# jongwon-jay-lee/llmss

Hardware: AMD Instinct MI355X
Metric: output_tokens_per_sec (higher is better)
Workload: dtype bf16

## Files before the change

### llmss_amd/csrc/common.h

```cpp
#pragma once
#include <hip/hip_runtime.h>
#include <hip/hip_bf16.h>
#include <stdint.h>
#include <algorithm>
#include <stdexcept>
#include <string>

#define LLMSS_WAVE 64

typedef unsigned short bf16_t;
typedef unsigned short __attribute__((ext_vector_type(8))) u16x8;
typedef unsigned short __attribute__((ext_vector_type(4))) u16x4;
typedef short __attribute__((ext_vector_type(8))) s16x8;
typedef short __attribute__((ext_vector_type(4))) s16x4;
typedef float __attribute__((ext_vector_type(4))) f32x4;
typedef float __attribute__((ext_vector_type(16))) f32x16;
typedef float __attribute__((ext_vector_type(2))) f32x2;
typedef unsigned int __attribute__((ext_vector_type(4))) u32x4;
typedef unsigned int __attribute__((ext_vector_type(2))) u32x2;

#define LDS_AS __attribute__((address_space(3)))

__device__ __forceinline__ float bf2f(bf16_t x) { return __uint_as_float(((unsigned)x) << 16); }

// ... 70 lines not shown
__device__ __forceinline__ float apply_act(float x, int act) {
  switch (act) {
    case ACT_GELU_TANH: return gelu_tanh(x);
    case ACT_GELU: return gelu_erf(x);
    case ACT_RELU: return fmaxf(x, 0.f);
    default: return x;
  }
}

__device__ __forceinline__ int xcd_remap(int orig, int nwg) {
  const int q = nwg >> 3, r = nwg & 7, xcd = orig & 7, idx = orig >> 3;
  return (xcd < r ? xcd * (q + 1) : r * (q + 1) + (xcd - r) * q) + idx;
}

__device__ __forceinline__ __amdgpu_buffer_rsrc_t uniform_rsrc(const void* p, int64_t bytes) {
  const uint64_t a = reinterpret_cast<uint64_t>(p);
  const uint32_t lo = __builtin_amdgcn_readfirstlane((uint32_t)a);
  const uint32_t hi = __builtin_amdgcn_readfirstlane((uint32_t)(a >> 32));
  const int n = __builtin_amdgcn_readfirstlane((int)(bytes < 0x7fffffff ? bytes : 0x7fffffff));
  return __builtin_amdgcn_make_buffer_rsrc(reinterpret_cast<void*>(((uint64_t)hi << 32) | lo), (short)0, n,
                                           0x00020000);
}

template <bool P32>
__device__ __forceinline__ f32x2 swap_pair(float x) {
  unsigned a = __builtin_bit_cast(unsigned, x), b = a;
  if constexpr (P32) asm volatile("s_nop 1\n\tv_permlane32_swap_b32 %0, %1" : "+v"(a), "+v"(b));
  else asm volatile("s_nop 1\n\tv_permlane16_swap_b32 %0, %1" : "+v"(a), "+v"(b));
  return f32x2{__builtin_bit_cast(float, a), __builtin_bit_cast(float, b)};
}
__device__ __forceinline__ float xor16_max(float x) { const f32x2 r = swap_pair<false>(x); return fmaxf(r[0], r[1]); }
__device__ __forceinline__ float xor32_max(float x) { const f32x2 r = swap_pair<true>(x); return fmaxf(r[0], r[1]); }
__device__ __forceinline__ float xor16_sum(float x) { const f32x2 r = swap_pair<false>(x); return r[0] + r[1]; }
__device__ __forceinline__ float xor32_sum(float x) { const f32x2 r = swap_pair<true>(x); return r[0] + r[1]; }

struct TileWork {
  int m0, n0, z;
};
__device__ __forceinline__ TileWork tile_work(int ntm, int ntn, int bm, int bn) {
  const int G = gridDim.x * gridDim.y;
  const int w = xcd_remap(blockIdx.y * gridDim.x + blockIdx.x, G);
  const int per = ntm * ntn;
  const int z = w / per, t = w - z * per;
  const int nt = t / ntm;
  return {(t - nt * ntm) * bm, nt * bn, z};
}

struct QkvEpi {
  const int64_t* pos;
  const float* cos_t;
  const float* sin_t;
  bf16_t* kc;
  bf16_t* vc;
  const int64_t* slot;
  int nh, nkv, D, rot, block_size, style, do_rope;
  unsigned char* mxq;
  unsigned char* mxs;
};

__device__ __forceinline__ int mx_block_exp(float amax) {
  const uint32_t b = __float_as_uint(amax / 448.f);
  int e = (int)((b >> 23) & 255) - 127 + ((b & 0x7fffffu) != 0u);
  return e < -126 ? -126 : (e > 126 ? 126 : e);
}

template <int BN>
struct EpiImg {
  static constexpr bool SWZ = BN % 32 == 0;
  static constexpr int LDW = SWZ ? BN : BN + 4;
  __device__ static __forceinline__ int at(int r, int c) { return r * LDW + (SWZ ? (c ^ (((r >> 2) & 1) << 4)) : c); }
  __device__ static __forceinline__ f32x4 ld4(const float* ct, int r, int c) {
    return *reinterpret_cast<const f32x4*>(ct + at(r, c));
  }
  __device__ static __forceinline__ void ld8(const float* ct, int r, int c, float (&x)[8]) {
    const int key = (threadIdx.x >> 3) & 1;
    const f32x4 a = ld4(ct, r, c + 4 * key), b = ld4(ct, r, c + 4 * (key ^ 1));
#pragma unroll
    for (int i = 0; i < 4; ++i) {
      x[i] = key ? b[i] : a[i];
      x[4 + i] = key ? a[i] : b[i];
    }
  }
};

template <int BN, int NTHR, int R>
__device__ __forceinline__ void qkv_store_chunk(const QkvEpi& e, const float* ct, int rows, int r0, int m0,
                                                int n0, int M, int N, bf16_t* __restrict__ Y, int64_t ldy,
                                                const bf16_t* __restrict__ bias) {
  constexpr int VPR = BN / 8, ITEMS = (R * VPR + NTHR - 1) / NTHR, G = ITEMS < 4 ? ITEMS : 4;
  const int D = e.D, nq = e.nh * D, nk = e.nkv * D, rh = e.rot >> 1;
  const bool rope = e.do_rope != 0;
#pragma unroll
  for (int i0 = 0; i0 < ITEMS; i0 += G) {
    int rr[G], cc[G], mm[G];
    bool ok[G];
    int64_t p[G], sl[G];
#pragma unroll
    for (int j = 0; j < G; ++j) {
      const int v = threadIdx.x + (i0 + j) * NTHR;
      rr[j] = v / VPR;
      cc[j] = (v - rr[j] * VPR) * 8;
      mm[j] = m0 + r0 + rr[j];
      ok[j] = i0 + j < ITEMS && rr[j] < rows && mm[j] < M && n0 + cc[j] < N;
      const int mc = min(mm[j], M - 1);
      p[j] = rope ? e.pos[mc] : 0;
      sl[j] = e.kc ? e.slot[mc] : -1;
    }
    f32x4 cs[G][2], sn[G][2];
#pragma unroll
    for (int j = 0; j < G; ++j) {
      if (rope) {
        const int n = n0 + cc[j], d = n % D;
        const bool lo = d < rh;
        int a = e.style == 1 ? (d >> 1) : (lo ? d : d - rh);
        a = (n < nq + nk && d < e.rot) ? a : 0;
        const float* cp = e.cos_t + p[j] * rh + a;
        const float* sp = e.sin_t + p[j] * rh + a;
        cs[j][0] = *reinterpret_cast<const f32x4*>(cp);
        sn[j][0] = *reinterpret_cast<const f32x4*>(sp);
        if (e.style != 1 && rh >= 8) {
          cs[j][1] = *reinterpret_cast<const f32x4*>(cp + 4);
          sn[j][1] = *reinterpret_cast<const f32x4*>(sp + 4);
        }
      }
    }
#pragma unroll
    for (int j = 0; j < G; ++j) {
      if (!ok[j]) continue;
      const int c = cc[j], n = n0 + c, d = n % D, m = mm[j];
      float x[8], y[8];
      EpiImg<BN>::ld8(ct, rr[j], c, x);
#pragma unroll
      for (int i = 0; i < 8; ++i) {
        x[i] = bf2f(f2bf(x[i] + (bias ? bf2f(bias[n + i]) : 0.f)));
        y[i] = x[i];
      }
      const bool is_v = n >= nq + nk;
      if (rope && !is_v && d < e.rot) {
        if (e.style == 1) {
#pragma unroll
          for (int i = 0; i < 4; ++i) {
            y[2 * i] = x[2 * i] * cs[j][0][i] - x[2 * i + 1] * sn[j][0][i];
            y[2 * i + 1] = x[2 * i + 1] * cs[j][0][i] + x[2 * i] * sn[j][0][i];
          }
        } else {
          const bool lo = d < rh;
          const int sh = lo ? rh : -rh;
          float xs[8];
          EpiImg<BN>::ld8(ct, rr[j], c + sh, xs);
#pragma unroll
          for (int i = 0; i < 8; ++i) {
            const float xp = bf2f(f2bf(xs[i] + (bias ? bf2f(bias[n + sh + i]) : 0.f)));
            const float cv = cs[j][i >> 2][i & 3], sv = sn[j][i >> 2][i & 3];
            y[i] = lo ? x[i] * cv - xp * sv : x[i] * cv + xp * sv;
          }
        }
      }
      u16x8 o;
#pragma unroll
      for (int i = 0; i < 8; ++i) o[i] = f2bf(y[i]);
      *reinterpret_cast<u16x8*>(Y + (int64_t)m * ldy + n) = o;
      if (n >= nq && sl[j] >= 0) {
        const int h = (n - (is_v ? nq + nk : nq)) / D;
        const int64_t row = ((sl[j] / e.block_size) * e.nkv + h) * (int64_t)e.block_size + sl[j] % e.block_size;
        *reinterpret_cast<u16x8*>((is_v ? e.vc : e.kc) + row * D + d) = o;
      }
    }
  }
}

template <int BN, int NTHR, int R>
__device__ __forceinline__ void img_store_rows(const float* ct, int rows, int r0, int m0, int n0, int M, int N,
                                               float* __restrict__ part, bf16_t* __restrict__ Y, int64_t ldy,
                                               const bf16_t* __restrict__ bias, int act, int glu, const QkvEpi& qe) {
  using Img = EpiImg<BN>;
  if (qe.D) {
    qkv_store_chunk<BN, NTHR, R>(qe, ct, rows, r0, m0, n0, M, N, Y, ldy, bias);
  } else if (part) {
    constexpr int VPR = BN / 4;
    for (int v = threadIdx.x; v < rows * VPR; v += NTHR) {
      const int r = v / VPR, c = (v - r * VPR) * 4;
      const int m = m0 + r0 + r, n = n0 + c;
      if (m >= M || n >= N) continue;
      const f32x4 val = Img::ld4(ct, r, c);
      float* dst = part + (int64_t)m * N + n;
      if (n + 3 < N && (N & 3) == 0) *reinterpret_cast<f32x4*>(dst) = val;
      else
        for (int j = 0; j < 4 && n + j < N; ++j) dst[j] = val[j];
    }
  } else if (glu && qe.mxq) {
    constexpr int VPR = BN / 16;
    static_assert(BN % 16 == 0, "SwiGLU tile");
    if constexpr (VPR % 4 == 0) {
      for (int v = threadIdx.x; v < rows * VPR; v += NTHR) {
        const int r = v / VPR, oc = (v - r * VPR) * 8;
        const int p = oc >> 4, j = oc & 15;
        const int cg = 32 * p + j, m = m0 + r0 + r, ng = n0 + cg;
        const bool ok = m < M && ng < N;
        float gx[8], ux[8], h[8];
        Img::ld8(ct, r, cg, gx);
        Img::ld8(ct, r, cg + 16, ux);
        float amax = 0.f;
#pragma unroll
        for (int e = 0; e < 8; ++e) {
          float gv = gx[e], uv = ux[e];
          if (bias && ok) { gv += bf2f(bias[ng + e]); uv += bf2f(bias[ng + 16 + e]); }
          h[e] = bf2f(f2bf(silu(gv) * uv));
          amax = fmaxf(amax, fabsf(h[e]));
        }
        amax = fmaxf(amax, __shfl_xor(amax, 1, 64));
        amax = fmaxf(amax, __shfl_xor(amax, 2, 64));
        const int ex = amax > 0.f ? mx_block_exp(amax) : 0;
        const float inv = __uint_as_float((uint32_t)(127 - ex) << 23);
        unsigned lo = 0, hi = 0;
        lo = __builtin_amdgcn_cvt_pk_fp8_f32(h[0] * inv, h[1] * inv, lo, false);
        lo = __builtin_amdgcn_cvt_pk_fp8_f32(h[2] * inv, h[3] * inv, lo, true);
        hi = __builtin_amdgcn_cvt_pk_fp8_f32(h[4] * inv, h[5] * inv, hi, false);
        hi = __builtin_amdgcn_cvt_pk_fp8_f32(h[6] * inv, h[7] * inv, hi, true);
        const int64_t oc_g = n0 / 2 + oc;
        if (ok) {
          *reinterpret_cast<uint2*>(qe.mxq + (int64_t)m * ldy + oc_g) = make_uint2(lo, hi);
          if ((v & 3) == 0) qe.mxs[(int64_t)m * (ldy / 32) + oc_g / 32] = (unsigned char)(ex + 127);
        }
      }
    }
  } else if (glu) {
    constexpr int VPR = BN / 16;
    for (int v = threadIdx.x; v < rows * VPR; v += NTHR) {
      const int r = v / VPR, oc = (v - r * VPR) * 8;
      const int p = oc >> 4, j = oc & 15;
      const int cg = 32 * p + j, m = m0 + r0 + r, ng = n0 + cg;
      if (m >= M || ng >= N) continue;
      u16x8 o;
      float gx[8], ux[8];
      Img::ld8(ct, r, cg, gx);
      Img::ld8(ct, r, cg + 16, ux);
#pragma unroll
      for (int e = 0; e < 8; ++e) {
        float gv = gx[e], uv = ux[e];
        if (bias) { gv += bf2f(bias[ng + e]); uv += bf2f(bias[ng + 16 + e]); }
        o[e] = f2bf(silu(gv) * uv);
      }
      bf16_t* dst = Y + (int64_t)m * ldy + n0 / 2 + oc;
      if (ng + 16 + 7 < N && (ldy & 7) == 0) *reinterpret_cast<u16x8*>(dst) = o;
      else
        for (int e = 0; e < 8 && ng + 16 + e < N; ++e) dst[e] = o[e];
    }
  } else {
    constexpr int VPR = BN / 8;
    for (int v = threadIdx.x; v < rows * VPR; v += NTHR) {
      const int r = v / VPR, c = (v - r * VPR) * 8;
      const int m = m0 + r0 + r, n = n0 + c;
      if (m >= M || n >= N) continue;
      u16x8 o;
      float xv[8];
      Img::ld8(ct, r, c, xv);
#pragma unroll
      for (int e = 0; e < 8; ++e) {
        float x = xv[e];
        if (bias && n + e < N) x += bf2f(bias[n + e]);
        o[e] = f2bf(apply_act(x, act));
      }
      bf16_t* dst = Y + (int64_t)m * ldy + n;
      if (n + 7 < N && (ldy & 7) == 0) *reinterpret_cast<u16x8*>(dst) = o;
      else
        for (int e = 0; e < 8 && n + e < N; ++e) dst[e] = o[e];
    }
  }
}

template <int BM, int BN, int MT, int NT, int NTHR, int LDSB>
__device__ __forceinline__ void tile_store_lds(const f32x4 (&acc)[MT][NT], char* lds, int wrow0, int wcol0, int m0,
                                               int n0, int M, int N, float* __restrict__ part,
                                               bf16_t* __restrict__ Y, int64_t ldy, const bf16_t* __restrict__ bias,
                                               int act, int glu, const QkvEpi& qe = QkvEpi{}) {
  using Img = EpiImg<BN>;
  constexpr int RMAX = LDSB / (Img::LDW * 4);
  constexpr int R = (RMAX >= BM ? BM : RMAX) / 16 * 16;
  static_assert(R >= 16, "LDS too small for a 16-row epilogue chunk");
  float* ct = reinterpret_cast<float*>(lds);
  const int lane = threadIdx.x & 63, li = lane & 15, g = lane >> 4;
  asm volatile("s_waitcnt lgkmcnt(0)" ::: "memory");
  __builtin_amdgcn_s_barrier();
  asm volatile("" ::: "memory");
  for (int r0 = 0; r0 < BM; r0 += R) {
#pragma unroll
    for (int mt = 0; mt < MT; ++mt) {
      const int rb = wrow0 + mt * 16;
      if (rb < r0 || rb >= r0 + R) continue;
#pragma unroll
      for (int i = 0; i < 4; ++i)
#pragma unroll
        for (int nt = 0; nt < NT; ++nt) ct[Img::at(rb - r0 + 4 * g + i, wcol0 + nt * 16 + li)] = acc[mt][nt][i];
    }
    asm volatile("s_waitcnt lgkmcnt(0)" ::: "memory");
    __builtin_amdgcn_s_barrier();
    asm volatile("" ::: "memory");
    const int rows = BM - r0 < R ? BM - r0 : R;
    img_store_rows<BN, NTHR, R>(ct, rows, r0, m0, n0, M, N, part, Y, ldy, bias, act, glu, qe);
    if (r0 + R < BM) {
      asm volatile("s_waitcnt lgkmcnt(0)" ::: "memory");
      __builtin_amdgcn_s_barrier();
      asm volatile("" ::: "memory");
    }
  }
}

template <int MT, int NT>
__device__ __forceinline__ bool splitk_combine(f32x4 (&acc)[MT][NT], float* ws, int* cnt, int tile, int S, int z,
                                               int wid, int nwaves, int lane, int* lds_word) {
  constexpr int G = MT * NT * 4 <= 32 ? 4 : (MT * NT * 4 <= 64 ? 2 : 1);
  const int tile_f = nwaves * MT * NT * 256;
  const auto rs = __builtin_amdgcn_make_buffer_rsrc(ws + (int64_t)tile * S * tile_f, (short)0,
                                                    (int)((uint32_t)S * (uint32_t)tile_f * 4u), 0x00020000);
  const uint32_t base = (uint32_t)((wid * MT * NT * 64 + lane) * 16);
  const uint32_t slab_b = (uint32_t)tile_f * 4u;
#pragma unroll
  for (int mt = 0; mt < MT; ++mt)
#pragma unroll
    for (int nt = 0; nt < NT; ++nt)
      __builtin_amdgcn_raw_buffer_store_b128(__builtin_bit_cast(u32x4, acc[mt][nt]), rs,
                                             base + (uint32_t)((mt * NT + nt) * 1024), (uint32_t)z * slab_b, 16);
  asm volatile("s_waitcnt vmcnt(0)" ::: "memory");
  __syncthreads();
  if (threadIdx.x == 0) *lds_word = __hip_atomic_fetch_add(cnt + tile, 1, __ATOMIC_RELAXED, __HIP_MEMORY_SCOPE_AGENT);
  __syncthreads();
  if (*lds_word != S - 1) return false;
  if (threadIdx.x == 0) __hip_atomic_store(cnt + tile, 0, __ATOMIC_RELAXED, __HIP_MEMORY_SCOPE_AGENT);
  __builtin_amdgcn_fence(__ATOMIC_ACQUIRE, "wavefront");
#pragma unroll
  for (int mt = 0; mt < MT; ++mt)
#pragma unroll
    for (int nt = 0; nt < NT; ++nt) acc[mt][nt] = f32x4{0.f, 0.f, 0.f, 0.f};
  for (int s0 = 0; s0 < S; s0 += G) {
    u32x4 v[G][MT][NT];
#pragma unroll
    for (int j = 0; j < G; ++j) {
      const uint32_t so = (uint32_t)min(s0 + j, S - 1) * slab_b;
#pragma unroll
      for (int mt = 0; mt < MT; ++mt)
#pragma unroll
        for (int nt = 0; nt < NT; ++nt)
          v[j][mt][nt] = __builtin_amdgcn_raw_buffer_load_b128(rs, base + (uint32_t)((mt * NT + nt) * 1024), so, 16);
// ... 24 lines not shown
```

### llmss_amd/csrc/gemm.hip

```cpp
#include "common.h"
#include "gemm_plan.h"

__device__ __forceinline__ void fp8x16_to_bf16(const u32x4& w, s16x8& f0, s16x8& f1) {
  const unsigned wd[4] = {w[0], w[1], w[2], w[3]};
  short o[16];
#pragma unroll
  for (int q = 0; q < 4; ++q) {
    f32x2 lo = __builtin_amdgcn_cvt_pk_f32_fp8(wd[q], false);
    f32x2 hi = __builtin_amdgcn_cvt_pk_f32_fp8(wd[q], true);
    o[4 * q + 0] = (short)f2bf(lo[0]);
    o[4 * q + 1] = (short)f2bf(lo[1]);
    o[4 * q + 2] = (short)f2bf(hi[0]);
    o[4 * q + 3] = (short)f2bf(hi[1]);
  }
  f0 = s16x8{o[0], o[1], o[2], o[3], o[4], o[5], o[6], o[7]};
  f1 = s16x8{o[8], o[9], o[10], o[11], o[12], o[13], o[14], o[15]};
}

__device__ __forceinline__ float epi_value(float v, int n, const float* wscale, const bf16_t* bias, int act) {
  if (wscale) v *= wscale[n];
  if (bias) v += bf2f(bias[n]);
  return apply_act(v, act);
}

// ... 276 lines not shown
    STREAM2_REM(w1, w0)
    STREAM2_REM(w2, w1)
    STREAM2_REM(w0, w2)
  } while (0);
#undef STREAM2_STEADY
#undef STREAM2_REM

#pragma unroll
  for (int mt = 0; mt < MT; ++mt) {
#pragma unroll
    for (int i = 0; i < 4; ++i) {
      const int m = mt * 16 + 4 * g + i;
      if (m >= M) continue;
      if (nsplit > 1) {
#pragma unroll
        for (int nt = 0; nt < NT; ++nt) {
          const int n = n0 + nt * 16 + li;
          if (n < N) part[((int64_t)split * M + m) * N + n] = acc[mt][nt][i] * (wscale ? wscale[n] : 1.f);
        }
      } else if (glu) {
#pragma unroll
        for (int p = 0; p < NT / 2; ++p) {
          const int ng = n0 + 2 * p * 16 + li, nu = ng + 16;
          if (nu < N) {
            const float gv = epi_value(acc[mt][2 * p][i], ng, wscale, bias, ACT_NONE);
            const float uv = epi_value(acc[mt][2 * p + 1][i], nu, wscale, bias, ACT_NONE);
            Y[(int64_t)m * ldy + n0 / 2 + p * 16 + li] = f2bf(silu(gv) * uv);
          }
        }
      } else {
#pragma unroll
        for (int nt = 0; nt < NT; ++nt) {
          const int n = n0 + nt * 16 + li;
          if (n < N) Y[(int64_t)m * ldy + n] = f2bf(epi_value(acc[mt][nt][i], n, wscale, bias, act));
        }
      }
    }
  }
}

__device__ __forceinline__ float slab_sum(const float* __restrict__ part, int S, int64_t stride, int64_t off) {
  constexpr int SG = 8;
  float v = 0.f;
  for (int s0 = 0; s0 < S; s0 += SG) {
    float x[SG];
#pragma unroll
    for (int g = 0; g < SG; ++g) x[g] = part[(int64_t)min(s0 + g, S - 1) * stride + off];
#pragma unroll
    for (int g = 0; g < SG; ++g) v += s0 + g < S ? x[g] : 0.f;
  }
  return v;
}

__global__ __launch_bounds__(256) void splitk_reduce_kernel(const float* __restrict__ part, int S, int M, int N,
                                                            const bf16_t* __restrict__ bias, bf16_t* __restrict__ Y,
                                                            int64_t ldy, int act, int glu) {
  const int m = blockIdx.y;
  const int nout = glu ? N / 2 : N;
  const int64_t stride = (int64_t)M * N;
  for (int c = blockIdx.x * blockDim.x + threadIdx.x; c < nout; c += gridDim.x * blockDim.x) {
    if (glu) {
      const int p = c >> 4, i = c & 15;
      const int ng = 32 * p + i, nu = ng + 16;
      float gv = slab_sum(part, S, stride, (int64_t)m * N + ng), uv = slab_sum(part, S, stride, (int64_t)m * N + nu);
      if (bias) { gv += bf2f(bias[ng]); uv += bf2f(bias[nu]); }
      Y[(int64_t)m * ldy + c] = f2bf(silu(gv) * uv);
    } else {
      float v = slab_sum(part, S, stride, (int64_t)m * N + c);
      if (bias) v += bf2f(bias[c]);
      Y[(int64_t)m * ldy + c] = f2bf(apply_act(v, act));
    }
  }
}

constexpr int TBK = 64;

template <int BN, bool F8, int NW = 4>
struct TiledB {
  static constexpr int ROWB = F8 ? 64 : 128;
  static constexpr int BYTES = BN * ROWB;
  static constexpr int LOADS = F8 ? BN / (16 * NW) : BN / (8 * NW);
};

template <int BM, int BN, bool WNT = false, bool F8 = false, int NW = 4>
__device__ __forceinline__ void tiled_stage(const bf16_t* __restrict__ A, int64_t lda, int M, const void* __restrict__ Bv,
                                            int64_t ldb, int N, int K, int m0, int n0, int k0, char* sA, char* sB,
                                            int w, int lane) {
  static_assert(BM % (8 * NW) == 0 && BN % (8 * NW) == 0, "tile rows must split evenly over the waves");
#pragma unroll
  for (int it = 0; it < BM / (8 * NW); ++it) {
    const int inst = it * NW + w;
    const int row = inst * 8 + (lane >> 3);
    const int c = (lane & 7) ^ (row & 7);
    const int kc = min(k0 + c * 8, K - 8);
    const bf16_t* ga = A + (int64_t)min(m0 + row, M - 1) * lda + kc;
    __builtin_amdgcn_global_load_lds((const void*)ga, (LDS_AS void*)(sA + inst * 1024), 16, 0, 0);
  }
  if constexpr (F8) {
    const unsigned char* B = reinterpret_cast<const unsigned char*>(Bv);
#pragma unroll
    for (int it = 0; it < BN / (16 * NW); ++it) {
      const int inst = it * NW + w;
      const int row = inst * 16 + (lane >> 2);
      const int gq = (lane & 3) ^ ((row >> 2) & 3);
      const int kc = min(k0 + gq * 16, K - 16);
      const unsigned char* gb = B + (int64_t)min(n0 + row, N - 1) * ldb + kc;
      __builtin_amdgcn_global_load_lds((const void*)gb, (LDS_AS void*)(sB + inst * 1024), 16, 0, WNT ? 2 : 0);
    }
  } else {
    const bf16_t* B = reinterpret_cast<const bf16_t*>(Bv);
#pragma unroll
    for (int it = 0; it < BN / (8 * NW); ++it) {
      const int inst = it * NW + w;
      const int row = inst * 8 + (lane >> 3);
      const int c = (lane & 7) ^ (row & 7);
      const int kc = min(k0 + c * 8, K - 8);
      const bf16_t* gb = B + (int64_t)min(n0 + row, N - 1) * ldb + kc;
      __builtin_amdgcn_global_load_lds((const void*)gb, (LDS_AS void*)(sB + inst * 1024), 16, 0, WNT ? 2 : 0);
    }
  }
}

template <int MTW, int NTW, bool MASK, bool F8 = false>
__device__ __forceinline__ void tiled_compute(const char* sA, const char* sB, f32x4 (&acc)[MTW][NTW], int wr, int wc,
                                              int li, int g, int k0, int K) {
#pragma unroll
  for (int s = 0; s < 2; ++s) {
    const int c = 4 * s + g;
    const bool valid = !MASK || (k0 + c * 8 < K);
    const s16x8 z = {0, 0, 0, 0, 0, 0, 0, 0};
    s16x8 a[MTW], b[NTW];
#pragma unroll
    for (int t = 0; t < MTW; ++t) {
      const int ra = wr * (MTW * 16) + t * 16 + li;
      a[t] = *reinterpret_cast<const s16x8*>(sA + ra * 128 + ((c ^ (ra & 7)) << 4));
      if (MASK && !valid) a[t] = z;
    }
#pragma unroll
    for (int t = 0; t < NTW; ++t) {
      const int rb = wc * (NTW * 16) + t * 16 + li;
      if constexpr (F8) {
        const int pq = (2 * s + (g >> 1)) ^ ((rb >> 2) & 3);
        const u32x2 raw = *reinterpret_cast<const u32x2*>(sB + rb * 64 + pq * 16 + (g & 1) * 8);
        b[t] = fp8x8_to_bf16(raw[0], raw[1]);
      } else {
        b[t] = *reinterpret_cast<const s16x8*>(sB + rb * 128 + ((c ^ (rb & 7)) << 4));
      }
      if (MASK && !valid) b[t] = z;
    }
#pragma unroll
    for (int mt = 0; mt < MTW; ++mt)
#pragma unroll
      for (int nt = 0; nt < NTW; ++nt)
        acc[mt][nt] = __builtin_amdgcn_mfma_f32_16x16x32_bf16(a[mt], b[nt], acc[mt][nt], 0, 0, 0);
  }
}

template <int N>
__device__ __forceinline__ void wait_vmcnt() {
  static_assert(N >= 0 && N < 64, "vmcnt range");
  asm volatile("s_waitcnt vmcnt(%0)" ::"n"(N) : "memory");
}

template <int LOADS, int MAXY>
__device__ __forceinline__ void wait_vmcnt_upto(int younger) {
  if constexpr (MAXY <= 0) {
    wait_vmcnt<0>();
  } else {
    if (younger >= MAXY) wait_vmcnt<LOADS * MAXY>();
    else wait_vmcnt_upto<LOADS, MAXY - 1>(younger);
  }
}

__device__ __forceinline__ void lds_barrier() {
  asm volatile("" ::: "memory");
  __builtin_amdgcn_s_waitcnt(0xC07F);
  __builtin_amdgcn_s_barrier();
  asm volatile("" ::: "memory");
}

template <int BM, int BN, int NS, bool WNT, bool F8 = false, int NW = 4>
__global__ __launch_bounds__(64 * NW) void gemm_tiled_kernel(const bf16_t* __restrict__ A, int64_t lda,
                                                         const void* __restrict__ B, int64_t ldb,
                                                         const bf16_t* __restrict__ bias, bf16_t* __restrict__ Y,
                                                         int64_t ldy, float* __restrict__ part, int M, int N, int K,
                                                         int act, int glu, const float* __restrict__ wscale,
                                                         int* __restrict__ cnt, QkvEpi qe) {
  constexpr int MTW = BM / (8 * NW), NTW = BN / 32;
  constexpr int A_BYTES = BM * TBK * 2, B_BYTES = TiledB<BN, F8, NW>::BYTES, STAGE = A_BYTES + B_BYTES;
  __shared__ __attribute__((aligned(16))) char smem[NS * STAGE];
  const int lane = threadIdx.x & 63;
  const int w = __builtin_amdgcn_readfirstlane(threadIdx.x >> 6);
  const int li = lane & 15, g = lane >> 4;
  const int wr = w >> 1, wc = w & 1;
  const int ntn = (N + BN - 1) / BN, ntm = (M + BM - 1) / BM;
  const TileWork tw = tile_work(ntm, ntn, BM, BN);
  const int m0 = tw.m0, n0 = tw.n0, zk = tw.z;

  f32x4 acc[MTW][NTW];
#pragma unroll
  for (int a = 0; a < MTW; ++a)
#pragma unroll
    for (int b = 0; b < NTW; ++b) acc[a][b] = f32x4{0.f, 0.f, 0.f, 0.f};

  const int nk_all = (K + TBK - 1) / TBK;
  const int per = (nk_all + gridDim.y - 1) / gridDim.y;
  const int t0 = zk * per, t1 = min(nk_all, t0 + per);
  if constexpr (NS == 2) {
    if (t0 < t1) {
      tiled_stage<BM, BN, WNT, F8, NW>(A, lda, M, B, ldb, N, K, m0, n0, t0 * TBK, smem, smem + A_BYTES, w, lane);
      asm volatile("s_waitcnt vmcnt(0)" ::: "memory");
      __syncthreads();
    }
    for (int t = t0; t < t1; ++t) {
      const int cur = (t - t0) & 1;
      char* nA = smem + (cur ^ 1) * STAGE;
      char* cA = smem + cur * STAGE;
      if (t + 1 < t1) tiled_stage<BM, BN, WNT, F8, NW>(A, lda, M, B, ldb, N, K, m0, n0, (t + 1) * TBK, nA, nA + A_BYTES, w, lane);
      if (t + 1 == nk_all && (K % TBK)) tiled_compute<MTW, NTW, true, F8>(cA, cA + A_BYTES, acc, wr, wc, li, g, t * TBK, K);
      else tiled_compute<MTW, NTW, false, F8>(cA, cA + A_BYTES, acc, wr, wc, li, g, t * TBK, K);
      asm volatile("s_waitcnt vmcnt(0)" ::: "memory");
      __syncthreads();
    }
  } else {
    constexpr int LOADS = BM / (8 * NW) + TiledB<BN, F8, NW>::LOADS;
#pragma unroll
    for (int j = 0; j < NS - 1; ++j)
      if (t0 + j < t1)
        tiled_stage<BM, BN, WNT, F8, NW>(A, lda, M, B, ldb, N, K, m0, n0, (t0 + j) * TBK, smem + j * STAGE,
                            smem + j * STAGE + A_BYTES, w, lane);
    int cur = 0;
    for (int t = t0; t < t1; ++t) {
      wait_vmcnt_upto<LOADS, NS - 2>(t1 - 1 - t);
      lds_barrier();
      char* cA = smem + cur * STAGE;
      const int nxt = cur == 0 ? NS - 1 : cur - 1;
      if (t + NS - 1 < t1) {
        char* nA = smem + nxt * STAGE;
        tiled_stage<BM, BN, WNT, F8, NW>(A, lda, M, B, ldb, N, K, m0, n0, (t + NS - 1) * TBK, nA, nA + A_BYTES, w, lane);
      }
      if (t + 1 == nk_all && (K % TBK)) tiled_compute<MTW, NTW, true, F8>(cA, cA + A_BYTES, acc, wr, wc, li, g, t * TBK, K);
      else tiled_compute<MTW, NTW, false, F8>(cA, cA + A_BYTES, acc, wr, wc, li, g, t * TBK, K);
      cur = cur == NS - 1 ? 0 : cur + 1;
    }
  }
  if (cnt) {
    asm volatile("s_waitcnt vmcnt(0)" ::: "memory");
    if (!splitk_combine<MTW, NTW>(acc, part, cnt, (n0 / BN) * ntm + m0 / BM, gridDim.y, zk, w, NW, lane,
                                  reinterpret_cast<int*>(smem)))
      return;
    part = nullptr;
  }
  if constexpr (!F8) {
    if (qe.D) {
      asm volatile("s_waitcnt vmcnt(0)" ::: "memory");
      tile_store_lds<BM, BN, MTW, NTW, 64 * NW, NS * STAGE>(acc, smem, wr * (MTW * 16), wc * (NTW * 16), m0, n0, M,
                                                             N, nullptr, Y, ldy, bias, act, glu, qe);
      return;
    }
  }
  const int wn0 = n0 + wc * (NTW * 16);
#pragma unroll
  for (int mt = 0; mt < MTW; ++mt) {
#pragma unroll
    for (int i = 0; i < 4; ++i) {
      const int m = m0 + wr * (MTW * 16) + mt * 16 + 4 * g + i;
      if (m >= M) continue;
      if (part) {
        float* pr = part + ((int64_t)zk * M + m) * N;
#pragma unroll
        for (int nt = 0; nt < NTW; ++nt) {
          const int n = wn0 + nt * 16 + li;
          if (n < N) pr[n] = F8 ? acc[mt][nt][i] * wscale[n] : acc[mt][nt][i];
        }
      } else if (glu) {
#pragma unroll
        for (int p = 0; p < NTW / 2; ++p) {
          const int ng = wn0 + 2 * p * 16 + li, nu = ng + 16;
          if (nu < N) {
            float gv = acc[mt][2 * p][i], uv = acc[mt][2 * p + 1][i];
            if constexpr (F8) { gv *= wscale[ng]; uv *= wscale[nu]; }
            if (bias) { gv += bf2f(bias[ng]); uv += bf2f(bias[nu]); }
            Y[(int64_t)m * ldy + wn0 / 2 + p * 16 + li] = f2bf(silu(gv) * uv);
          }
        }
      } else {
#pragma unroll
        for (int nt = 0; nt < NTW; ++nt) {
          const int n = wn0 + nt * 16 + li;
          if (n < N) {
            float v = acc[mt][nt][i];
            if constexpr (F8) v *= wscale[n];
            if (bias) v += bf2f(bias[n]);
            Y[(int64_t)m * ldy + n] = f2bf(apply_act(v, act));
          }
        }
      }
    }
  }
}

static int g_big_group_m = 4;
void gemm_big_set_group(int g) { g_big_group_m = g >= 1 && g <= 64 ? g : 4; }

__device__ __forceinline__ f32x4 mfma_f8x2(s16x8 a0, s16x8 a1, s16x8 b0, s16x8 b1, f32x4 c) {
  typedef int __attribute__((ext_vector_type(4))) i32x4_t;
  typedef int __attribute__((ext_vector_type(8))) i32x8_t;
  const i32x4_t al = __builtin_bit_cast(i32x4_t, a0), ah = __builtin_bit_cast(i32x4_t, a1);
  const i32x4_t bl = __builtin_bit_cast(i32x4_t, b0), bh = __builtin_bit_cast(i32x4_t, b1);
  const i32x8_t av = __builtin_shufflevector(al, ah, 0, 1, 2, 3, 4, 5, 6, 7);
  const i32x8_t bv = __builtin_shufflevector(bl, bh, 0, 1, 2, 3, 4, 5, 6, 7);
  return __builtin_amdgcn_mfma_scale_f32_16x16x128_f8f6f4(av, bv, c, 0, 0, 0, 127, 0, 127);
}

template <bool F8>
__global__ __launch_bounds__(512, 1) void gemm_big_kernel(const void* __restrict__ A, int64_t lda,
                                                          const void* __restrict__ B, int64_t ldb,
                                                          const bf16_t* __restrict__ bias, bf16_t* __restrict__ Y,
                                                          int64_t ldy, int M, int N, int K, int act, int glu,
                                                          const float* __restrict__ xs, const float* __restrict__ ws,
                                                          int group_m) {
  constexpr int ES = F8 ? 1 : 2;
  constexpr int HALF = 16384, BUF = 4 * HALF;
  __shared__ __attribute__((aligned(16))) char smem[2 * BUF];
  const int lane = threadIdx.x & 63;
  const int w = __builtin_amdgcn_readfirstlane(threadIdx.x >> 6);
  const int li = lane & 15, g = lane >> 4;
  const int wr = w >> 2, wc = w & 3;
  const int ntn = (N + 255) / 256, ntm = (M + 255) / 256;
  const int GM = group_m;
  const int tile = xcd_remap(blockIdx.x, ntn * ntm);
  const int grp = tile / (GM * ntn), gidx = tile - grp * (GM * ntn);
  const int gm = min(GM, ntm - grp * GM);
  const int m0 = (grp * GM + gidx % gm) * 256, n0 = (gidx / gm) * 256;
  const int nk = K * ES / 128;

  const char* src[4] = {(const char*)A, (const char*)A, (const char*)B, (const char*)B};
  const int64_t ld[4] = {lda * ES, lda * ES, ldb * ES, ldb * ES};
  int64_t soff[4][2];
  int lofs[2];
#pragma unroll
// ... 854 lines not shown
```

### llmss_amd/csrc/gemm_dec.hip

```cpp
#include "common.h"
#include "gemm_plan.h"

namespace {

template <int MT, int BN, int NSW>
struct DecCfg {
  static constexpr int NW = 4;
  static constexpr int NT = BN / 16;
  static constexpr int AR = MT * 16;
  static constexpr int AL = AR / 8, BL = BN / 8;
  static constexpr int LOADS = AL + BL;
  static constexpr int SLOT = (AR + BN) * 128;
  static constexpr int RING = NW * NSW * SLOT;
  static constexpr int RED = NW * MT * NT * 1024;
  static constexpr int IMG = AR * EpiImg<BN>::LDW * 4;
  static constexpr int LDS = RING > RED + IMG ? RING : RED + IMG;
  static constexpr bool FITS = LDS <= 160 * 1024;
};

template <int N_>
__device__ __forceinline__ void dec_wait(int younger_stages) {
  if (younger_stages >= 3) asm volatile("s_waitcnt vmcnt(%0)" ::"n"(3 * N_) : "memory");
  else if (younger_stages == 2) asm volatile("s_waitcnt vmcnt(%0)" ::"n"(2 * N_) : "memory");
  else if (younger_stages == 1) asm volatile("s_waitcnt vmcnt(%0)" ::"n"(N_) : "memory");
// ... 41 lines not shown
__global__ __launch_bounds__(256) void gemm_dec_kernel(const bf16_t* __restrict__ A, int64_t lda,
                                                       const bf16_t* __restrict__ B, int64_t ldb,
                                                       const bf16_t* __restrict__ bias, bf16_t* __restrict__ Y,
                                                       int64_t ldy, float* __restrict__ part, int M, int N, int K,
                                                       int act, int glu, QkvEpi qe, int* __restrict__ cnt) {
  using C = DecCfg<MT, BN, NSW>;
  static_assert(BN % 16 == 0 && C::BL >= 1, "BN: multiple of 16");
  static_assert(3 * C::LOADS <= 63, "vmcnt immediate");
  static_assert(C::FITS, "LDS");
  constexpr int NW = C::NW, NT = C::NT, AR = C::AR, AL = C::AL, BL = C::BL, LOADS = C::LOADS, SLOT = C::SLOT;
  __shared__ __attribute__((aligned(16))) char smem[C::LDS];

  const int lane = threadIdx.x & 63;
  const int w = __builtin_amdgcn_readfirstlane(threadIdx.x >> 6);
  const int li = lane & 15, g = lane >> 4;
  const int ntn = (N + BN - 1) / BN;
  const TileWork tw = tile_work(1, ntn, AR, BN);
  const int n0 = tw.n0, zk = tw.z;

  const int nk_all = (K + 63) / 64;
  const int per = (nk_all + gridDim.y - 1) / gridDim.y;
  const int t0 = zk * per, t1 = min(nk_all, t0 + per);
  const int mine = t1 - t0 - w;
  const int nloc = mine > 0 ? (mine + NW - 1) / NW : 0;
  const bool ktail = (K & 63) != 0;

  const uint64_t abytes = (uint64_t)M * (uint64_t)lda * 2;
  const uint64_t bbytes = PK ? (uint64_t)((N + 15) / 16 - n0 / 16) * (uint64_t)nk_all * 2048
                             : (uint64_t)(N - n0) * (uint64_t)ldb * 2;
  const int64_t bbase = PK ? (int64_t)(n0 / 16) * nk_all * 2048 : (int64_t)n0 * ldb * 2;
  const auto ra = __builtin_amdgcn_make_buffer_rsrc(const_cast<char*>(reinterpret_cast<const char*>(A)), (short)0,
                                                    (int)(abytes > 0xFFFFFFF0ull ? 0xFFFFFFF0u : (uint32_t)abytes),
                                                    0x00020000);
  const auto rb = __builtin_amdgcn_make_buffer_rsrc(const_cast<char*>(reinterpret_cast<const char*>(B) + bbase),
                                                    (short)0,
                                                    (int)(bbytes > 0xFFFFFFF0ull ? 0xFFFFFFF0u : (uint32_t)bbytes),
                                                    0x00020000);
  uint32_t va[AL], vb[BL];
#pragma unroll
  for (int i = 0; i < AL; ++i) {
    const int row = i * 8 + (lane >> 3);
    va[i] = (uint32_t)(row * lda * 2 + (((lane & 7) ^ (row & 7)) << 4));
  }
#pragma unroll
  for (int i = 0; i < BL; ++i) {
    const int row = i * 8 + (lane >> 3);
    vb[i] = (PK ? (uint32_t)((row >> 4) * nk_all * 2048 + (row & 15) * 128) : (uint32_t)(row * ldb * 2)) +
            (uint32_t)(((lane & 7) ^ (row & 7)) << 4);
  }
  char* ring = smem + w * (NSW * SLOT);

#define DEC_ISSUE(J_)                                                                                            \
  do {                                                                                                           \
    const int t_ = t0 + w + NW * (J_);                                                                           \
    char* sl_ = ring + ((J_) % NSW) * SLOT;                                                                      \
    const uint32_t so_ = (uint32_t)t_ * 128u, sob_ = (uint32_t)t_ * (PK ? 2048u : 128u);                         \
    if (MODE == 3) {                                                                                             \
    } else if (!ktail || t_ != nk_all - 1) {                                                                     \
      if (MODE != 1) _Pragma("unroll") for (int i_ = 0; i_ < AL; ++i_)                                           \
        __builtin_amdgcn_raw_ptr_buffer_load_lds(ra, (LDS_AS void*)(sl_ + i_ * 1024), 16, (uint32_t)va[i_],      \
                                                 (uint32_t)so_, 0, 0);                                           \
      if (MODE != 2) _Pragma("unroll") for (int i_ = 0; i_ < BL; ++i_)     \
        __builtin_amdgcn_raw_ptr_buffer_load_lds(rb, (LDS_AS void*)(sl_ + AR * 128 + i_ * 1024), 16,             \
                                                 (uint32_t)vb[i_], (uint32_t)sob_, 0, 2);                         \
    } else {          \
      _Pragma("unroll") for (int i_ = 0; i_ < AL; ++i_)                                                          \
        __builtin_amdgcn_raw_ptr_buffer_load_lds(ra, (LDS_AS void*)(sl_ + i_ * 1024), 16,                        \
                                                 (uint32_t)(va[i_] + so_), (uint32_t)0, 0, 0);                   \
      _Pragma("unroll") for (int i_ = 0; i_ < BL; ++i_)                                                          \
        __builtin_amdgcn_raw_ptr_buffer_load_lds(rb, (LDS_AS void*)(sl_ + AR * 128 + i_ * 1024), 16,             \
                                                 (uint32_t)(vb[i_] + sob_), (uint32_t)0, 0, 2);                  \
    }                                                                                                            \
  } while (0)

  f32x4 acc[MT][NT];
#pragma unroll
  for (int a = 0; a < MT; ++a)
#pragma unroll
    for (int b = 0; b < NT; ++b) acc[a][b] = f32x4{0.f, 0.f, 0.f, 0.f};

  const int x0 = (g ^ (li & 7)) << 4, x1 = ((4 + g) ^ (li & 7)) << 4;
  const int fa = li * 128, fb = AR * 128 + li * 128;

  const int pre = nloc < NSW ? nloc : NSW;
  for (int j = 0; j < pre; ++j) DEC_ISSUE(j);
  for (int j = 0; j < nloc; ++j) {
    const int younger = min(NSW - 1, nloc - 1 - j);
    if constexpr (MODE == 0 || MODE == 4) dec_wait<LOADS>(younger);
    else if constexpr (MODE == 1) dec_wait<BL>(younger);
    else if constexpr (MODE == 2) dec_wait<AL>(younger);
    const char* st = ring + (j % NSW) * SLOT;
    const int t = t0 + w + NW * j;
    if (ktail && t == nk_all - 1) {
      const int kv = K - t * 64;
      char* sw = const_cast<char*>(st);
      for (int idx = lane; idx < AR * 8; idx += 64) {
        const int row = idx >> 3, c = idx & 7;
        if (c * 8 >= kv) *reinterpret_cast<u32x4*>(sw + row * 128 + ((c ^ (row & 7)) << 4)) = u32x4{0u, 0u, 0u, 0u};
      }
      asm volatile("s_waitcnt lgkmcnt(0)" ::: "memory");
    }
#pragma unroll
    for (int s = 0; s < 2; ++s) {
      const int xo = s ? x1 : x0;
      s16x8 a[MT], b[NT];
#pragma unroll
      for (int mt = 0; mt < MT; ++mt) a[mt] = *reinterpret_cast<const s16x8*>(st + fa + mt * 2048 + xo);
#pragma unroll
      for (int nt = 0; nt < NT; ++nt) b[nt] = *reinterpret_cast<const s16x8*>(st + fb + nt * 2048 + xo);
#pragma unroll
      for (int mt = 0; mt < MT; ++mt)
#pragma unroll
        for (int nt = 0; nt < NT; ++nt)
          acc[mt][nt] = __builtin_amdgcn_mfma_f32_16x16x32_bf16(a[mt], b[nt], acc[mt][nt], 0, 0, 0);
    }
    if (j + NSW < nloc) {
      asm volatile("s_waitcnt lgkmcnt(0)" ::: "memory");
      DEC_ISSUE(j + NSW);
    }
  }

#undef DEC_ISSUE

  asm volatile("s_waitcnt vmcnt(0) lgkmcnt(0)" ::: "memory");
  __builtin_amdgcn_s_barrier();
  asm volatile("" ::: "memory");
  f32x4* red = reinterpret_cast<f32x4*>(smem);
#pragma unroll
  for (int mt = 0; mt < MT; ++mt)
#pragma unroll
    for (int nt = 0; nt < NT; ++nt) red[((w * MT + mt) * NT + nt) * 64 + lane] = acc[mt][nt];
  asm volatile("s_waitcnt lgkmcnt(0)" ::: "memory");
  __builtin_amdgcn_s_barrier();
  asm volatile("" ::: "memory");
  using Img = EpiImg<BN>;
  float* ct = reinterpret_cast<float*>(smem + C::RED);
#pragma unroll
  for (int q = 0; q < MT * NT; ++q) {
    if (q % NW != w) continue;
    const int mt = q / NT, nt = q % NT;
    f32x4 v = red[(mt * NT + nt) * 64 + lane];
#pragma unroll
    for (int u = 1; u < NW; ++u) {
      const f32x4 p = red[((u * MT + mt) * NT + nt) * 64 + lane];
#pragma unroll
      for (int i = 0; i < 4; ++i) v[i] += p[i];
    }
#pragma unroll
    for (int i = 0; i < 4; ++i) ct[Img::at(mt * 16 + 4 * g + i, nt * 16 + li)] = v[i];
  }
  asm volatile("s_waitcnt lgkmcnt(0)" ::: "memory");
  __builtin_amdgcn_s_barrier();
  asm volatile("" ::: "memory");
  if constexpr (MODE == 4) {
    if (M < 0) part[threadIdx.x] = ct[threadIdx.x];
    return;
  }
  if (cnt) {
    if (!dec_combine<BN, AR>(ct, part, cnt, n0 / BN, gridDim.y, zk, reinterpret_cast<int*>(smem))) return;
    part = nullptr;
  }
  img_store_rows<BN, 64 * NW, AR>(ct, AR, 0, 0, n0, M, N, part ? part + (int64_t)zk * M * N : nullptr, Y, ldy, bias,
                                  act, glu, qe);
}

template <int MT, int BN, int NS>
static void dec_launch(dim3 grid, hipStream_t st, const bf16_t* X, int64_t ldx, const bf16_t* W, int64_t ldw,
                       const bf16_t* bias, bf16_t* Y, int64_t ldy, float* part, int M, int N, int K, int act, int glu,
                       const QkvEpi& qv, int* cnt, bool packed) {
  if constexpr (NS > 2 && !DecCfg<MT, BN, NS>::FITS) {
    dec_launch<MT, BN, NS - 1>(grid, st, X, ldx, W, ldw, bias, Y, ldy, part, M, N, K, act, glu, qv, cnt, packed);
  } else if (packed) {
    gemm_dec_kernel<MT, BN, NS, 0, true><<<grid, 256, 0, st>>>(X, ldx, W, ldw, bias, Y, ldy, part, M, N, K, act, glu,
                                                               qv, cnt);
  } else {
    gemm_dec_kernel<MT, BN, NS><<<grid, 256, 0, st>>>(X, ldx, W, ldw, bias, Y, ldy, part, M, N, K, act, glu, qv, cnt);
  }
}

static int dec_depth(int mt, int bn, int want) {
  int ns = std::max(2, std::min(want, 4));
  const int slot = (mt * 16 + bn) * 128;
  while (ns > 2 && 4 * ns * slot > 160 * 1024) --ns;
  return ns;
}

void launch_gemm_dec(int code, int depth, const bf16_t* X, int64_t ldx, const bf16_t* W, int64_t ldw,
                     const bf16_t* bias, bf16_t* Y, int64_t ldy, float* part, int M, int N, int K, int act, int glu,
                     int split, hipStream_t st, const QkvEpi* qe, int* cnt, bool packed = false) {
  const GemmTile* tile = gemm_tile(code, true);
  if (!tile) throw std::runtime_error("gemm_dec: bad tile code");
  const int bn = tile->bn;
  if (M < 1 || M > 64) throw std::runtime_error("gemm_dec: M must be 1..64");
  if (glu && (bn % 32)) throw std::runtime_error("gemm_dec: SwiGLU needs 32-column tile pairs");
  if ((uint64_t)64 * ldx * 2 >= (1ull << 31) || (!packed && (uint64_t)bn * ldw * 2 >= (1ull << 31)) ||
      (packed && (uint64_t)(bn / 16 + 1) * ((K + 63) / 64) * 2048 >= (1ull << 31)))
    throw std::runtime_error("gemm_dec: row stride too large for 32-bit buffer offsets");
  const int mt = M <= 16 ? 1 : (M <= 32 ? 2 : 4);
  const int ns = dec_depth(mt, bn, depth);
  const QkvEpi qv = qe ? *qe : QkvEpi{};
  dim3 grid((N + bn - 1) / bn, split);
#define DECN(MT_, BN_)                                                                                           \
  do {                                                                                                           \
    if (ns >= 4) dec_launch<MT_, BN_, 4>(grid, st, X, ldx, W, ldw, bias, Y, ldy, part, M, N, K, act, glu, qv, cnt, packed);   \
    else if (ns == 3) dec_launch<MT_, BN_, 3>(grid, st, X, ldx, W, ldw, bias, Y, ldy, part, M, N, K, act, glu, qv, cnt, packed); \
    else dec_launch<MT_, BN_, 2>(grid, st, X, ldx, W, ldw, bias, Y, ldy, part, M, N, K, act, glu, qv, cnt, packed);          \
  } while (0)
#define DECB(MT_)                                                                                                \
  do {                                                                                                           \
    switch (bn) {                                                                                                \
      case 16: DECN(MT_, 16); break;                                                                             \
      case 32: DECN(MT_, 32); break;                                                                             \
      case 48: DECN(MT_, 48); break;                                                                             \
      case 64: DECN(MT_, 64); break;                                                                             \
      default: DECN(MT_, 96); break;                                                                             \
    }                                                                                                            \
  } while (0)
  if (mt == 1) DECB(1);
  else if (mt == 2) DECB(2);
  else DECB(4);
#undef DECB
#undef DECN
  HIP_CHECK_LAUNCH();
}
```

Before: 12540.

## Prefetch QKV rope/position data, reorder decode LDS reads, add tiled split-K LDS epilogue

Splits the fused QKV epilogue so that position/slot indices load before the decode GEMM main loop and cos/sin tables load before the reduction barrier, which hides their global-load latency. The decode K-loop now reads both halves of the LDS fragments before issuing the next async stage, so the refill overlaps the MFMA work. Bias loads in the GLU and plain epilogues are hoisted ahead of the LDS reads. The tiled GEMM gains a MODE template parameter for probing A-only, B-only or compute-only variants, plus an LDS-staged split-K partial store for BM=64. The cost is more live registers and extra template instantiations.

```diff
diff --git a/llmss_amd/csrc/common.h b/llmss_amd/csrc/common.h
--- a/llmss_amd/csrc/common.h
+++ b/llmss_amd/csrc/common.h
@@ -176,6 +176,121 @@
     }
   }
 };
+
+template <int BN, int NTHR, int R>
+struct QkvGeom {
+  static constexpr int VPR = BN / 8, ITEMS = (R * VPR + NTHR - 1) / NTHR, G = ITEMS < 4 ? ITEMS : 4;
+};
+
+template <int G>
+struct QkvPre {
+  int64_t p[G], sl[G];
+  f32x4 cs[G][2], sn[G][2];
+};
+
+template <int BN, int NTHR, int R>
+__device__ __forceinline__ void qkv_load_pos(const QkvEpi& e, int i0, int r0, int m0, int M,
+                                             QkvPre<QkvGeom<BN, NTHR, R>::G>& q) {
+  constexpr int VPR = QkvGeom<BN, NTHR, R>::VPR, G = QkvGeom<BN, NTHR, R>::G;
+  const bool rope = e.do_rope != 0;
+#pragma unroll
+  for (int j = 0; j < G; ++j) {
+    const int v = threadIdx.x + (i0 + j) * NTHR;
+    const int mc = min(m0 + r0 + v / VPR, M - 1);
+    q.p[j] = rope ? e.pos[mc] : 0;
+    q.sl[j] = e.kc ? e.slot[mc] : -1;
+  }
+}
+
+template <int BN, int NTHR, int R>
+__device__ __forceinline__ void qkv_load_trig(const QkvEpi& e, int i0, int n0, QkvPre<QkvGeom<BN, NTHR, R>::G>& q) {
+  constexpr int VPR = QkvGeom<BN, NTHR, R>::VPR, G = QkvGeom<BN, NTHR, R>::G;
+  const int D = e.D, nq = e.nh * D, nk = e.nkv * D, rh = e.rot >> 1;
+  if (!e.do_rope) return;
+#pragma unroll
+  for (int j = 0; j < G; ++j) {
+    const int v = threadIdx.x + (i0 + j) * NTHR;
+    const int n = n0 + (v - (v / VPR) * VPR) * 8, d = n % D;
+    const bool lo = d < rh;
+    int a = e.style == 1 ? (d >> 1) : (lo ? d : d - rh);
+    a = (n < nq + nk && d < e.rot) ? a : 0;
+    const float* cp = e.cos_t + q.p[j] * rh + a;
+    const float* sp = e.sin_t + q.p[j] * rh + a;
+    q.cs[j][0] = *reinterpret_cast<const f32x4*>(cp);
+    q.sn[j][0] = *reinterpret_cast<const f32x4*>(sp);
+    if (e.style != 1 && rh >= 8) {
+      q.cs[j][1] = *reinterpret_cast<const f32x4*>(cp + 4);
+      q.sn[j][1] = *reinterpret_cast<const f32x4*>(sp + 4);
+    }
+  }
+}
+
+template <int BN, int NTHR, int R>
+__device__ __forceinline__ void qkv_store_items(const QkvEpi& e, const float* ct, int rows, int i0, int r0, int m0,
+                                                int n0, int M, int N, bf16_t* __restrict__ Y, int64_t ldy,
+                                                const bf16_t* __restrict__ bias,
+                                                const QkvPre<QkvGeom<BN, NTHR, R>::G>& q) {
+  constexpr int VPR = QkvGeom<BN, NTHR, R>::VPR, ITEMS = QkvGeom<BN, NTHR, R>::ITEMS, G = QkvGeom<BN, NTHR, R>::G;
+  const int D = e.D, nq = e.nh * D, nk = e.nkv * D, rh = e.rot >> 1;
+  const bool rope = e.do_rope != 0;
+  const auto& cs = q.cs;
+  const auto& sn = q.sn;
+  const auto& sl = q.sl;
+  {
+    int rr[G], cc[G], mm[G];
+    bool ok[G];
+#pragma unroll
+    for (int j = 0; j < G; ++j) {
+      const int v = threadIdx.x + (i0 + j) * NTHR;
+      rr[j] = v / VPR;
+      cc[j] = (v - rr[j] * VPR) * 8;
+      mm[j] = m0 + r0 + rr[j];
+      ok[j] = i0 + j < ITEMS && rr[j] < rows && mm[j] < M && n0 + cc[j] < N;
+    }
+#pragma unroll
+    for (int j = 0; j < G; ++j) {
+      if (!ok[j]) continue;
+      const int c = cc[j], n = n0 + c, d = n % D, m = mm[j];
+      float x[8], y[8];
+      EpiImg<BN>::ld8(ct, rr[j], c, x);
+#pragma unroll
+      for (int i = 0; i < 8; ++i) {
+        x[i] = bf2f(f2bf(x[i] + (bias ? bf2f(bias[n + i]) : 0.f)));
+        y[i] = x[i];
+      }
+      const bool is_v = n >= nq + nk;
+      if (rope && !is_v && d < e.rot) {
+        if (e.style == 1) {
+#pragma unroll
+          for (int i = 0; i < 4; ++i) {
+            y[2 * i] = x[2 * i] * cs[j][0][i] - x[2 * i + 1] * sn[j][0][i];
+            y[2 * i + 1] = x[2 * i + 1] * cs[j][0][i] + x[2 * i] * sn[j][0][i];
+          }
+        } else {
+          const bool lo = d < rh;
+          const int sh = lo ? rh : -rh;
+          float xs[8];
+          EpiImg<BN>::ld8(ct, rr[j], c + sh, xs);
+#pragma unroll
+          for (int i = 0; i < 8; ++i) {
+            const float xp = bf2f(f2bf(xs[i] + (bias ? bf2f(bias[n + sh + i]) : 0.f)));
+            const float cv = cs[j][i >> 2][i & 3], sv = sn[j][i >> 2][i & 3];
+            y[i] = lo ? x[i] * cv - xp * sv : x[i] * cv + xp * sv;
+          }
+        }
+      }
+      u16x8 o;
+#pragma unroll
+      for (int i = 0; i < 8; ++i) o[i] = f2bf(y[i]);
+      *reinterpret_cast<u16x8*>(Y + (int64_t)m * ldy + n) = o;
+      if (n >= nq && sl[j] >= 0) {
+        const int h = (n - (is_v ? nq + nk : nq)) / D;
+        const int64_t row = ((sl[j] / e.block_size) * e.nkv + h) * (int64_t)e.block_size + sl[j] % e.block_size;
+        *reinterpret_cast<u16x8*>((is_v ? e.vc : e.kc) + row * D + d) = o;
+      }
+    }
+  }
+}
 
 template <int BN, int NTHR, int R>
 __device__ __forceinline__ void qkv_store_chunk(const QkvEpi& e, const float* ct, int rows, int r0, int m0,
@@ -326,13 +441,17 @@
       const int cg = 32 * p + j, m = m0 + r0 + r, ng = n0 + cg;
       if (m >= M || ng >= N) continue;
       u16x8 o;
-      float gx[8], ux[8];
+      float gx[8], ux[8], bg[8], bu[8];
+      if (bias) {
+#pragma unroll
+        for (int e = 0; e < 8; ++e) { bg[e] = bf2f(bias[ng + e]); bu[e] = bf2f(bias[ng + 16 + e]); }
+      }
       Img::ld8(ct, r, cg, gx);
       Img::ld8(ct, r, cg + 16, ux);
 #pragma unroll
       for (int e = 0; e < 8; ++e) {
         float gv = gx[e], uv = ux[e];
-        if (bias) { gv += bf2f(bias[ng + e]); uv += bf2f(bias[ng + 16 + e]); }
+        if (bias) { gv += bg[e]; uv += bu[e]; }
         o[e] = f2bf(silu(gv) * uv);
       }
       bf16_t* dst = Y + (int64_t)m * ldy + n0 / 2 + oc;
@@ -347,12 +466,16 @@
       const int m = m0 + r0 + r, n = n0 + c;
       if (m >= M || n >= N) continue;
       u16x8 o;
-      float xv[8];
+      float xv[8], bv[8];
+      if (bias) {
+#pragma unroll
+        for (int e = 0; e < 8; ++e) bv[e] = bf2f(bias[min(n + e, N - 1)]);
+      }
       Img::ld8(ct, r, c, xv);
 #pragma unroll
       for (int e = 0; e < 8; ++e) {
         float x = xv[e];
-        if (bias && n + e < N) x += bf2f(bias[n + e]);
+        if (bias && n + e < N) x += bv[e];
         o[e] = f2bf(apply_act(x, act));
       }
       bf16_t* dst = Y + (int64_t)m * ldy + n;
diff --git a/llmss_amd/csrc/gemm.hip b/llmss_amd/csrc/gemm.hip
--- a/llmss_amd/csrc/gemm.hip
+++ b/llmss_amd/csrc/gemm.hip
@@ -382,13 +382,13 @@
   static constexpr int LOADS = F8 ? BN / (16 * NW) : BN / (8 * NW);
 };
 
-template <int BM, int BN, bool WNT = false, bool F8 = false, int NW = 4>
+template <int BM, int BN, bool WNT = false, bool F8 = false, int NW = 4, int MODE = 0>
 __device__ __forceinline__ void tiled_stage(const bf16_t* __restrict__ A, int64_t lda, int M, const void* __restrict__ Bv,
                                             int64_t ldb, int N, int K, int m0, int n0, int k0, char* sA, char* sB,
                                             int w, int lane) {
   static_assert(BM % (8 * NW) == 0 && BN % (8 * NW) == 0, "tile rows must split evenly over the waves");
 #pragma unroll
-  for (int it = 0; it < BM / (8 * NW); ++it) {
+  for (int it = 0; it < (MODE == 1 || MODE == 3 ? 0 : BM / (8 * NW)); ++it) {
     const int inst = it * NW + w;
     const int row = inst * 8 + (lane >> 3);
     const int c = (lane & 7) ^ (row & 7);
@@ -396,7 +396,8 @@
     const bf16_t* ga = A + (int64_t)min(m0 + row, M - 1) * lda + kc;
     __builtin_amdgcn_global_load_lds((const void*)ga, (LDS_AS void*)(sA + inst * 1024), 16, 0, 0);
   }
-  if constexpr (F8) {
+  if constexpr (MODE == 2 || MODE == 3) {
+  } else if constexpr (F8) {
     const unsigned char* B = reinterpret_cast<const unsigned char*>(Bv);
 #pragma unroll
     for (int it = 0; it < BN / (16 * NW); ++it) {
@@ -479,7 +480,7 @@
   asm volatile("" ::: "memory");
 }
 
-template <int BM, int BN, int NS, bool WNT, bool F8 = false, int NW = 4>
+template <int BM, int BN, int NS, bool WNT, bool F8 = false, int NW = 4, int MODE = 0>
 __global__ __launch_bounds__(64 * NW) void gemm_tiled_kernel(const bf16_t* __restrict__ A, int64_t lda,
                                                          const void* __restrict__ B, int64_t ldb,
                                                          const bf16_t* __restrict__ bias, bf16_t* __restrict__ Y,
@@ -508,7 +509,7 @@
   const int t0 = zk * per, t1 = min(nk_all, t0 + per);
   if constexpr (NS == 2) {
     if (t0 < t1) {
-      tiled_stage<BM, BN, WNT, F8, NW>(A, lda, M, B, ldb, N, K, m0, n0, t0 * TBK, smem, smem + A_BYTES, w, lane);
+      tiled_stage<BM, BN, WNT, F8, NW, MODE>(A, lda, M, B, ldb, N, K, m0, n0, t0 * TBK, smem, smem + A_BYTES, w, lane);
       asm volatile("s_waitcnt vmcnt(0)" ::: "memory");
       __syncthreads();
     }
@@ -516,18 +517,19 @@
       const int cur = (t - t0) & 1;
       char* nA = smem + (cur ^ 1) * STAGE;
       char* cA = smem + cur * STAGE;
-      if (t + 1 < t1) tiled_stage<BM, BN, WNT, F8, NW>(A, lda, M, B, ldb, N, K, m0, n0, (t + 1) * TBK, nA, nA + A_BYTES, w, lane);
+      if (t + 1 < t1) tiled_stage<BM, BN, WNT, F8, NW, MODE>(A, lda, M, B, ldb, N, K, m0, n0, (t + 1) * TBK, nA, nA + A_BYTES, w, lane);
       if (t + 1 == nk_all && (K % TBK)) tiled_compute<MTW, NTW, true, F8>(cA, cA + A_BYTES, acc, wr, wc, li, g, t * TBK, K);
       else tiled_compute<MTW, NTW, false, F8>(cA, cA + A_BYTES, acc, wr, wc, li, g, t * TBK, K);
       asm volatile("s_waitcnt vmcnt(0)" ::: "memory");
       __syncthreads();
     }
   } else {
-    constexpr int LOADS = BM / (8 * NW) + TiledB<BN, F8, NW>::LOADS;
+    constexpr int LOADS = (MODE == 1 || MODE == 3 ? 0 : BM / (8 * NW)) +
+                          (MODE == 2 || MODE == 3 ? 0 : TiledB<BN, F8, NW>::LOADS);
 #pragma unroll
     for (int j = 0; j < NS - 1; ++j)
       if (t0 + j < t1)
-        tiled_stage<BM, BN, WNT, F8, NW>(A, lda, M, B, ldb, N, K, m0, n0, (t0 + j) * TBK, smem + j * STAGE,
+        tiled_stage<BM, BN, WNT, F8, NW, MODE>(A, lda, M, B, ldb, N, K, m0, n0, (t0 + j) * TBK, smem + j * STAGE,
                             smem + j * STAGE + A_BYTES, w, lane);
     int cur = 0;
     for (int t = t0; t < t1; ++t) {
@@ -537,7 +539,7 @@
       const int nxt = cur == 0 ? NS - 1 : cur - 1;
       if (t + NS - 1 < t1) {
         char* nA = smem + nxt * STAGE;
-        tiled_stage<BM, BN, WNT, F8, NW>(A, lda, M, B, ldb, N, K, m0, n0, (t + NS - 1) * TBK, nA, nA + A_BYTES, w, lane);
+        tiled_stage<BM, BN, WNT, F8, NW, MODE>(A, lda, M, B, ldb, N, K, m0, n0, (t + NS - 1) * TBK, nA, nA + A_BYTES, w, lane);
       }
       if (t + 1 == nk_all && (K % TBK)) tiled_compute<MTW, NTW, true, F8>(cA, cA + A_BYTES, acc, wr, wc, li, g, t * TBK, K);
       else tiled_compute<MTW, NTW, false, F8>(cA, cA + A_BYTES, acc, wr, wc, li, g, t * TBK, K);
@@ -551,12 +553,29 @@
       return;
     part = nullptr;
   }
+  if constexpr (MODE == 4) {
+    float keep = 0.f;
+#pragma unroll
+    for (int a = 0; a < MTW; ++a)
+#pragma unroll
+      for (int b = 0; b < NTW; ++b) keep += acc[a][b][0] + acc[a][b][1] + acc[a][b][2] + acc[a][b][3];
+    if (M < 0) part[threadIdx.x] = keep;
+    return;
+  }
   if constexpr (!F8) {
     if (qe.D) {
       asm volatile("s_waitcnt vmcnt(0)" ::: "memory");
       tile_store_lds<BM, BN, MTW, NTW, 64 * NW, NS * STAGE>(acc, smem, wr * (MTW * 16), wc * (NTW * 16), m0, n0, M,
                                                              N, nullptr, Y, ldy, bias, act, glu, qe);
       return;
+    }
+    if constexpr (BM == 64) {
+      if (part) {
+        asm volatile("s_waitcnt vmcnt(0)" ::: "memory");
+        tile_store_lds<BM, BN, MTW, NTW, 64 * NW, NS * STAGE>(acc, smem, wr * (MTW * 16), wc * (NTW * 16), m0, n0, M,
+                                                               N, part + (int64_t)zk * M * N, Y, ldy, bias, act, glu);
+        return;
+      }
     }
   }
   const int wn0 = n0 + wc * (NTW * 16);
diff --git a/llmss_amd/csrc/gemm_dec.hip b/llmss_amd/csrc/gemm_dec.hip
--- a/llmss_amd/csrc/gemm_dec.hip
+++ b/llmss_amd/csrc/gemm_dec.hip
@@ -147,6 +147,11 @@
   const int x0 = (g ^ (li & 7)) << 4, x1 = ((4 + g) ^ (li & 7)) << 4;
   const int fa = li * 128, fb = AR * 128 + li * 128;
 
+  using QG = QkvGeom<BN, 64 * NW, AR>;
+  static_assert(QG::ITEMS <= QG::G, "one QkvPre holds the whole tile");
+  QkvPre<QG::G> qpre;
+  if (qe.D) qkv_load_pos<BN, 64 * NW, AR>(qe, 0, 0, 0, M, qpre);
+
   const int pre = nloc < NSW ? nloc : NSW;
   for (int j = 0; j < pre; ++j) DEC_ISSUE(j);
   for (int j = 0; j < nloc; ++j) {
@@ -165,29 +170,30 @@
       }
       asm volatile("s_waitcnt lgkmcnt(0)" ::: "memory");
     }
+    s16x8 a[2][MT], b[2][NT];
 #pragma unroll
     for (int s = 0; s < 2; ++s) {
       const int xo = s ? x1 : x0;
-      s16x8 a[MT], b[NT];
-#pragma unroll
-      for (int mt = 0; mt < MT; ++mt) a[mt] = *reinterpret_cast<const s16x8*>(st + fa + mt * 2048 + xo);
-#pragma unroll
-      for (int nt = 0; nt < NT; ++nt) b[nt] = *reinterpret_cast<const s16x8*>(st + fb + nt * 2048 + xo);
+#pragma unroll
+      for (int mt = 0; mt < MT; ++mt) a[s][mt] = *reinterpret_cast<const s16x8*>(st + fa + mt * 2048 + xo);
+#pragma unroll
+      for (int nt = 0; nt < NT; ++nt) b[s][nt] = *reinterpret_cast<const s16x8*>(st + fb + nt * 2048 + xo);
+    }
+    asm volatile("s_waitcnt lgkmcnt(0)" ::: "memory");
+    if (j + NSW < nloc) DEC_ISSUE(j + NSW);
+#pragma unroll
+    for (int s = 0; s < 2; ++s)
 #pragma unroll
       for (int mt = 0; mt < MT; ++mt)
 #pragma unroll
         for (int nt = 0; nt < NT; ++nt)
-          acc[mt][nt] = __builtin_amdgcn_mfma_f32_16x16x32_bf16(a[mt], b[nt], acc[mt][nt], 0, 0, 0);
-    }
-    if (j + NSW < nloc) {
-      asm volatile("s_waitcnt lgkmcnt(0)" ::: "memory");
-      DEC_ISSUE(j + NSW);
-    }
+          acc[mt][nt] = __builtin_amdgcn_mfma_f32_16x16x32_bf16(a[s][mt], b[s][nt], acc[mt][nt], 0, 0, 0);
   }
 
 #undef DEC_ISSUE
 
   asm volatile("s_waitcnt vmcnt(0) lgkmcnt(0)" ::: "memory");
+  if (qe.D) qkv_load_trig<BN, 64 * NW, AR>(qe, 0, n0, qpre);
   __builtin_amdgcn_s_barrier();
   asm volatile("" ::: "memory");
   f32x4* red = reinterpret_cast<f32x4*>(smem);
@@ -225,8 +231,10 @@
     if (!dec_combine<BN, AR>(ct, part, cnt, n0 / BN, gridDim.y, zk, reinterpret_cast<int*>(smem))) return;
     part = nullptr;
   }
-  img_store_rows<BN, 64 * NW, AR>(ct, AR, 0, 0, n0, M, N, part ? part + (int64_t)zk * M * N : nullptr, Y, ldy, bias,
-                                  act, glu, qe);
+  if (qe.D) qkv_store_items<BN, 64 * NW, AR>(qe, ct, AR, 0, 0, 0, n0, M, N, Y, ldy, bias, qpre);
+  else
+    img_store_rows<BN, 64 * NW, AR>(ct, AR, 0, 0, n0, M, N, part ? part + (int64_t)zk * M * N : nullptr, Y, ldy, bias,
+                                    act, glu, qe);
 }
 
 template <int MT, int BN, int NS>
```

New measurement: 12560, median of 3. About the same (+0.2%).
